# zitongbai/bipedal_control

Hardware: AMD Instinct MI355X
Metric: MPC solves/s (H1, horizon=100) (higher is better)
Workload: dtype f64; 1 GPU; Unitree H1 trot (template tiled from t = 0), horizon=100 intervals (dt 0.015), batch=256 per GPU perturbed initial states, cold start, 1 SQP iteration (BASELINE.json configs[1]); solver=sqp, global_batch=256, problems_on_rank0=256, shooting_nodes=108, nx=22, nu=22

## Files before the change

bipedal_control_amd/csrc/k_node.hip:

```cpp
#include <hip/hip_runtime.h>
#include <hip/hip_ext.h>

#include <stdexcept>

#include "kernel_launchers.h"
#include "launch.h"
#include "kernels/rollout.h"

namespace bpmpc {

template <int NJ>
__global__ __launch_bounds__(kWave) void k_prepare(Launch L) {
  constexpr int NX = 12 + NJ, NU = 12 + NJ;
  const int s = blockIdx.x, b = s / L.N, k = s % L.N;
  const int g = L.buf.p_grid[b];
  const int n = L.buf.g_nodes[g];
  if (k >= n) { if (threadIdx.x == 0) L.buf.n_info[s] = 0; return; }
  const size_t gs = (size_t)g * L.N + k;
  if (threadIdx.x == 0) L.buf.n_info[s] = 8 | ((L.buf.g_mode[gs] & 3) << 1) | (L.buf.g_kind[gs] == 1 ? 1 : 0);
  if (threadIdx.x < kNodeAux) {
    const int t = threadIdx.x;
    L.buf.n_aux[(size_t)s * kNodeAux + t] = t == 0 ? L.buf.g_dt[gs] : t < 5 ? L.buf.g_zref[gs * 4 + t - 1] : t < 9 ? L.buf.g_zdref[gs * 4 + t - 5] : 0.0;
  }
  prepare_node<NJ>(*L.model, L.buf.g_kind[gs], L.buf.g_mode[gs], L.buf.g_start[gs], L.cold != 0, k == n - 1, L.buf.p_tgt_n[b],
// ... 11 lines not shown
  if (k >= L.buf.g_nodes[L.buf.p_grid[b]]) return;
  const size_t s = sidx;
  const NodeInputs in = node_inputs<NJ>(L, b, k);
  NodeLQOut out;
  out.A = L.buf.A + s * NX * NX; out.B = L.buf.B + s * NX * NU; out.b = L.buf.b + s * NX;
  out.Q = L.buf.Q + s * NX * NX; out.R = L.buf.R + s * NU * NU; out.P = L.buf.P + s * NU * NX;
  out.q = L.buf.q + s * NX; out.r = L.buf.r + s * NU; out.c = L.buf.c + s;
  out.C = L.buf.C + s * kMaxEqRows * NX; out.D = L.buf.D + s * kMaxEqRows * NU; out.e = L.buf.e + s * kMaxEqRows;
  out.nc = L.buf.nc + s; out.perf = L.buf.perf + s * 3;
  out.prof = (b == 0 && k < 64) ? L.buf.rprof + 8 * k : nullptr;
  linearize_node<NJ>(*L.model, ws, in, out, L.ilqr != 0, L.ilqr_shift);
}

constexpr int kTrialWaves = 4;
template <int NJ> constexpr int lin_waves() { return 4; }
template <int NJ, bool MAT, bool CHAIN, bool ILQR = false>
__global__ __launch_bounds__(lin_waves<NJ>() * kWave) __attribute__((amdgpu_waves_per_eu(2, 2))) void k_linearize_fast(Launch L) {
  using C = LinFastCfg<NJ, true, CHAIN>;
  constexpr int LPN = C::LPN, NPW = C::NPW, kLinWaves = lin_waves<NJ>();
  constexpr bool PARK = sizeof(LinFastNodeLds<NJ, true, CHAIN, true>) * (kLinWaves * NPW) + sizeof(LinFastShared<NJ>) <= 80 * 1024;
  using NL = LinFastNodeLds<NJ, true, CHAIN, PARK>;
  __shared__ NL lds[kLinWaves * NPW];
  __shared__ LinFastShared<NJ> shared;
#ifdef BPMPC_LIN_TIMELINE
  const long long tl0 = wall_clock64();
#endif
  const int sub = threadIdx.x / LPN, g = threadIdx.x % LPN;
  const int widx = blockIdx.x * (kLinWaves * NPW) + sub;
  bool valid, event_wg = false;
  int b, k;
  if (L.lin_ev_n >= 0) {
    constexpr int per_wg = kLinWaves * NPW;
// ... 38 lines not shown
#endif
  valid = valid && act != 0 && info != 0;
  const size_t s = valid ? (size_t)b * L.N + k : 0;
  LinFastOut out;
  out.A = L.buf.A; out.B = L.buf.B; out.b = L.buf.b; out.Q = L.buf.Q; out.R = L.buf.R; out.q = L.buf.q; out.r = L.buf.r; out.c = L.buf.c;
  out.C = L.buf.C; out.D = L.buf.D; out.e = L.buf.e; out.perf = L.buf.perf; out.nc = L.buf.nc;
  out.park = L.buf.lin_park;
  out.dump = L.buf.lin_dump;
  out.qrd = L.buf.qrd;
  out.s = s;
  out.ilqr_shift = L.ilqr_shift;
#ifndef BPMPC_LIN_PROF_PROBLEM
#define BPMPC_LIN_PROF_PROBLEM 0
#endif
  out.prof = (valid && b == BPMPC_LIN_PROF_PROBLEM && k < 64) ? L.buf.rprof + 8 * k : nullptr;
  linearize_fast<NJ, MAT, C, NL, ILQR>(*L.model, shared, lds[sub], valid, in, pre, out, g);
#ifdef BPMPC_LIN_TIMELINE
  if (threadIdx.x % kWave == 0 && blockIdx.x < 2048) {
    double* t = L.buf.rprof + 16 * blockIdx.x + 4 * (threadIdx.x / kWave);
    unsigned hw; asm volatile("s_getreg_b32 %0, hwreg(HW_REG_HW_ID)" : "=s"(hw));
    unsigned xcc; asm volatile("s_getreg_b32 %0, hwreg(HW_REG_XCC_ID)" : "=s"(xcc));
    t[0] = (double)tl0; t[1] = (double)tl1; t[2] = (double)wall_clock64(); t[3] = (double)(hw | ((unsigned long long)(xcc & 15) << 32));
  }
#endif
}

template <int NJ>
__global__ __launch_bounds__(kWave) void k_warm_shift(Launch L, const int* restarted) {
  constexpr int NX = 12 + NJ, NU = 12 + NJ;
  __shared__ double xi[NX];
  __shared__ double Ks[2][NU * NX];
  const int b = blockIdx.x / L.N, i = blockIdx.x % L.N, l = threadIdx.x;
  const int N = L.N;
  if (restarted && restarted[b]) return;
  const int g = L.buf.p_grid[b], n = L.buf.g_nodes[g];
  if (i >= n) return;
  const int gp = L.buf.tp_grid[b], np = L.buf.tp_nodes[gp];
  if (np < 1) return;
  const double* tp = L.buf.tp_time + (size_t)gp * (N + 1);
// ... 198 lines not shown
  const size_t i0 = (size_t)blockIdx.x * blockDim.x + threadIdx.x, stride = (size_t)gridDim.x * blockDim.x;
  const double2* a2 = reinterpret_cast<const double2*>(a_src);
  const double2* b2 = reinterpret_cast<const double2*>(b_src);
  double2* ad = reinterpret_cast<double2*>(a_dst);
  double2* bd = reinterpret_cast<double2*>(b_dst);
  for (size_t i = i0; i < na / 2; i += stride) ad[i] = a2[i];
  for (size_t i = i0; i < nb / 2; i += stride) bd[i] = b2[i];
  if (i0 == 0) { if (na & 1) a_dst[na - 1] = a_src[na - 1]; if (nb & 1) b_dst[nb - 1] = b_src[nb - 1]; }
  if (iterations) for (size_t i = i0; i < (size_t)batch; i += stride) { iterations[i] = 0; active[i] = 1; }
}

namespace kl {

void prepare(int nj, int slots, hipStream_t st, const Launch& L) { KL_NJ(nj, hipLaunchKernelGGL(k_prepare<NJ>, dim3(slots), dim3(kWave), 0, st, L)); }
void linearize_reference(int nj, int slots, hipStream_t st, const Launch& L) { KL_NJ(nj, hipLaunchKernelGGL(k_linearize<NJ>, dim3(slots), dim3(kWave), 0, st, L)); }
void linearize_fast(int nj, bool materialise, int nodes, hipStream_t st, const Launch& L, hipEvent_t ev_start, hipEvent_t ev_stop) {
  KL_NJ(nj, {
    constexpr int per_wg = lin_waves<NJ>() * LinFastCfg<NJ, true>::NPW;
    const int wgs = L.lin_ev_n >= 0 ? (L.batch * L.lin_inter + per_wg - 1) / per_wg + (L.batch * L.lin_ev_n + per_wg - 1) / per_wg : (nodes + per_wg - 1) / per_wg;
    const dim3 grid(wgs), block(lin_waves<NJ>() * kWave);
    auto launch = [&](auto kernel) {
      if (ev_start && ev_stop) hipExtLaunchKernelGGL(kernel, grid, block, 0, st, ev_start, ev_stop, 0, L);
      else hipLaunchKernelGGL(kernel, grid, block, 0, st, L);
    };
    if (L.ilqr) {
      if (!L.serial_legs) throw std::runtime_error("linearize_fast: the ILQR lineariser is instantiated for serial-leg robots only");
      if (materialise) launch(k_linearize_fast<NJ, true, true, true>);
      else launch(k_linearize_fast<NJ, false, true, true>);
    } else if (L.serial_legs) {
      if (materialise) launch(k_linearize_fast<NJ, true, true>);
      else launch(k_linearize_fast<NJ, false, true>);
    } else {
      if (materialise) launch(k_linearize_fast<NJ, true, false>);
      else launch(k_linearize_fast<NJ, false, false>);
    }
  });
}
void warm_shift(int nj, int slots, hipStream_t st, const Launch& L, const int* restarted) {
  KL_NJ(nj, hipLaunchKernelGGL(k_warm_shift<NJ>, dim3(slots), dim3(kWave), 0, st, L, restarted));
}
void ls_begin(int nj, int batch, hipStream_t st, const Launch& L) { KL_NJ(nj, hipLaunchKernelGGL(k_ls_begin<NJ>, dim3(batch), dim3(kWave), 0, st, L)); }
void trial_reference(int nj, int slots, hipStream_t st, const Launch& L) { KL_NJ(nj, hipLaunchKernelGGL(k_trial<NJ>, dim3(slots), dim3(kWave), 0, st, L)); }
int trial_fast_workgroups(int nj, int nodes) {
  const int per_wg = kTrialWaves * (nj == 10 ? LinFastCfg<10, true>::NPW : LinFastCfg<12, true>::NPW);
  return (nodes + per_wg - 1) / per_wg;
}
void trial_fast(int nj, int nodes, hipStream_t st, const Launch& L) {
  const int grid = trial_fast_workgroups(nj, nodes);
  KL_NJ(nj, {
    if (L.serial_legs) hipLaunchKernelGGL((k_trial_fast<NJ, true>), dim3(grid), dim3(kTrialWaves * kWave), 0, st, L);
    else hipLaunchKernelGGL((k_trial_fast<NJ, false>), dim3(grid), dim3(kTrialWaves * kWave), 0, st, L);
  });
// ... 33 lines not shown
```

bipedal_control_amd/csrc/kernels/linearize_fast.h:

```cpp
#pragma once
#include <hip/hip_runtime.h>

#include "node_lq.h"
#include "riccati_fast.h"

namespace bpmpc {

template <int NJ, bool PACK = false, bool CHAIN_ = false>
struct LinFastCfg {
  static constexpr bool CHAIN = CHAIN_;
  static constexpr int LEG = NJ / 2;
  static constexpr int NB = NJ + 1, G = 6 + NJ, NX = 12 + NJ, NU = 12 + NJ;
  static constexpr int G0 = (PACK && G > 16 && G - 3 <= 16) ? 3 : 0;
  static constexpr int LPN = (G - G0 <= 16) ? 16 : 32;
  static constexpr int NPW = kWave / LPN;
};

struct LinFastScalars {
  double contact_off[kNumContacts][3];
  double friction, cone_reg, cone_grip, cone_shift, barrier_mu, barrier_delta, pos_gain, robot_mass;
  unsigned contact_path[kNumContacts];
  int contact_body[kNumContacts];
  int max_depth, cone_gauss_newton;
};
// ... 494 lines not shown
      acc[0] += d[1] * Fi[2] - d[2] * Fi[1];
      acc[1] += d[2] * Fi[0] - d[0] * Fi[2];
      acc[2] += d[0] * Fi[1] - d[1] * Fi[0];
    }
    const double imt = 1.0 / mass_total;
    for (int r = 0; r < 3; ++r) ev.ar_q[r] = acc[r] * imt;
  }
  }
  EVPROF(7);
}

constexpr int kLinParkDoublesPerLane = 15;
constexpr int kLinDumpNodes = 1024, kLinDumpSlack = 1024;
constexpr size_t kLinDumpDoubles = (size_t)kLinDumpNodes * 16 + kLinDumpSlack;
constexpr int kQrdStride = 40;
constexpr int kQrdRShift = 37;
constexpr int kNodeAux = 16;
constexpr int kMaxDdpSteps = 16;

struct LinFastPre {
  double x0, x1, u0, u1, xn_q, xn_h, xn_t, xr_q, xr_h, xr_t;
  double aux;
};
template <class Cfg>
__device__ __forceinline__ LinFastPre linearize_preload(const double* x, const double* xnext, const double* u, const double* xref, int ln, const double* aux = nullptr) {
  constexpr int G = Cfg::G, NX = Cfg::NX, G0 = Cfg::G0;
  const int g = ln + G0;
  const bool tr = G0 > 0 && ln < 3;
  LinFastPre p;
  p.aux = (aux && ln < kNodeAux) ? aux[ln] : 0.0;
  p.x0 = x[ln]; p.u0 = u[ln];
// ... 22 lines not shown
  static_assert(Cfg::LPN == 16 && (PACKED || Cfg::G == 16), "role slots are laid out for sixteen lanes per node");
  int ln, g;
  double* dump;
  __device__ __forceinline__ void pointers(double* Xn, double* Un, double* (&p)[NS]) const {
    if constexpr (!PACKED) {
      p[0] = Xn + (6 + ln);
      p[1] = ln < 6 ? Xn + ln : Un + (12 + ln - 6);
      p[2] = ln < 12 ? Un + ln : dump;
    } else {
      p[0] = g < Cfg::G ? Xn + (6 + g) : dump;
      p[1] = ln < 3 ? Xn + (6 + ln) : (g < Cfg::G ? Un + (12 + g - 6) : dump);
      p[2] = ln < 12 ? Un + ln : dump;
      p[3] = ln < 6 ? Xn + ln : dump;
    }
  }
  __device__ __forceinline__ void store(double* const (&p)[NS], int off, double v_coord, double v_trans, double v_mom, double v_force, double v_joint) const {
    p[0][off] = v_coord;
    if constexpr (!PACKED) {
      p[1][off] = ln < 6 ? v_mom : v_joint;
      p[2][off] = v_force;
    } else {
      p[1][off] = ln < 3 ? v_trans : v_joint;
      p[2][off] = v_force;
      p[3][off] = v_mom;
    }
  }
};

template <int NJ, bool MAT = true, class Cfg = LinFastCfg<NJ, true>, class NL = LinFastNodeLds<NJ, true, Cfg::CHAIN, false>, bool ILQR = false>
__device__ __forceinline__ void linearize_fast(const DeviceModel& md, const LinFastShared<NJ>& sh, NL& nl, bool valid,
                                               const NodeInputs& in, const LinFastPre& pre, const LinFastOut& o, int ln) {
#ifdef BPMPC_LINFAST_PROFILE
  long long lf_t[8] = {0, 0, 0, 0, 0, 0, 0, 0};
  long long lf_prev = clock64();
  const long long lf_wall0 = wall_clock64(), lf_c0 = lf_prev;
#define LFPROF(slot) do { const long long tn_ = clock64(); lf_t[slot] += tn_ - lf_prev; lf_prev = tn_; } while (0)
#else
#define LFPROF(slot) ((void)0)
#endif
  using C = Cfg;
  constexpr int G = C::G, NX = C::NX, NU = C::NU, LPN = C::LPN, G0 = C::G0;
  constexpr bool PACKED = G0 > 0;
  const int g = ln + G0;
  const bool tr = PACKED && ln < 3;
  if (!valid) return;
  if (in.kind == 1) {
    double d2 = 0.0;
    if constexpr (MAT) {
      for (int idx = ln; idx < NX * NX; idx += LPN) { (o.A + o.s * (NX * NX))[idx] = (idx / NX == idx % NX) ? 1.0 : 0.0; (o.Q + o.s * (NX * NX))[idx] = 0.0; }
      for (int idx = ln; idx < NX * NU; idx += LPN) { (o.B + o.s * (NX * NU))[idx] = 0.0; }
      for (int idx = ln; idx < NU * NU; idx += LPN) (o.R + o.s * (NU * NU))[idx] = 0.0;
      for (int idx = ln; idx < kMaxEqRows * NX; idx += LPN) (o.C + o.s * (kMaxEqRows * NX))[idx] = 0.0;
      for (int idx = ln; idx < kMaxEqRows * NU; idx += LPN) (o.D + o.s * (kMaxEqRows * NU))[idx] = 0.0;
      for (int idx = ln; idx < kMaxEqRows; idx += LPN) (o.e + o.s * (kMaxEqRows))[idx] = 0.0;
    }
    {
      static_assert(LPN == 16 && NX <= 32, "two elements of x per lane");
      const double xq_lo = __shfl(pre.x0, (6 + g) & 15, LPN), xq_hi = __shfl(pre.x1, (6 + g - 16) & 15, LPN);
      const double xq = 6 + g < 16 ? xq_lo : xq_hi;
      const double xt = __shfl(pre.x0, (6 + ln) & 15, LPN);
      if (g < G) { const double d = ILQR ? 0.0 : xq - pre.xn_q; (o.b + o.s * (NX))[6 + g] = d; d2 += d * d; }
      if (ln < 6) { const double d = ILQR ? 0.0 : pre.x0 - pre.xn_h; (o.b + o.s * (NX))[ln] = d; d2 += d * d; }
      if (tr) { const double d = ILQR ? 0.0 : xt - pre.xn_t; (o.b + o.s * (NX))[6 + ln] = d; d2 += d * d; }
      if constexpr (MAT) for (int idx = ln; idx < NX; idx += LPN) { (o.q + o.s * (NX))[idx] = 0.0; (o.r + o.s * (NU))[idx] = 0.0; }
    }
    d2 = node_allreduce_add<LPN>(d2);
// ... 178 lines not shown
    for (int rr = 3; rr < 9; ++rr) c1j[rr] = is_joint ? nl.park[9 + rr - 3][ln] : 0.0;
  } else {
    const double* pk = o.park + o.s * (15 * LPN);
    for (int rr = 0; rr < 9; ++rr) c1q[rr] = pk[rr * LPN + ln];
    for (int rr = 0; rr < 9; ++rr) c1j[rr] = 0.0;
    if (is_joint) for (int rr = 3; rr < 9; ++rr) c1j[rr] = pk[9 * LPN + (rr - 3) * LPN + ln];
  }
  for (int rr = 0; rr < 9; ++rr) {
    c1h[rr] = momentum_col(nl.X12[0], nl.X22[0], imt, mass_total, ln, rr);
    c1f[rr] = force_col(nl.cps[0], nl.com[0], imt, ln, rr);
  }
  {
    double* pab[NS];
    slots.pointers(o.A + o.s * (NX * NX), o.B + o.s * (NX * NU), pab);
#pragma unroll
    for (int r = MAT ? 0 : 3; r < (MAT ? NX : 12); ++r) {
      double aq, ah_, bf, bj;
      if (r < 3 || r >= 12) {
        aq = (r == 6 + g) ? 1.0 : 0.0;
        ah_ = (r == ln) ? 1.0 : 0.0;
        bf = (r < 3 && (ln % 3) == r) ? dt * imt : 0.0;
        bj = (r >= 12 && r == 12 + g - 6) ? dt : 0.0;
      } else if constexpr (ILQR) {
        const int rr = r - 3;
        aq = ((r == 6 + g) ? 1.0 : 0.0) + dt * c1q[rr];
        ah_ = ((r == ln) ? 1.0 : 0.0) + dt * c1h[rr];
        bf = dt * c1f[rr];
        bj = dt * c1j[rr];
      } else {
        const int rr = r - 3;
        double sq = 0.0, sh = 0.0, sf = 0.0, sj = 0.0;
        for (int l = 0; l < 9; ++l) {
          const double a = nl.a2[rr][3 + l];
          sq += a * c1q[l]; sh += a * c1h[l]; sf += a * c1f[l]; sj += a * c1j[l];
        }
        sf += nl.a2[rr][ln % 3] * imt;
        sj += e2.ar_q[rr];
        const double e2h = momentum_col(nl.X12[1], nl.X22[1], imt, mass_total, ln, rr);
        const double e2f = force_col(nl.cps[1], nl.com[1], imt, ln, rr);
        const double e2j = rr < 3 ? 0.0 : e2.br_j[rr - 3];
        aq = ((r == 6 + g) ? 1.0 : 0.0) + hdt * (c1q[rr] + e2.ar_q[rr] + dt * sq);
        ah_ = ((r == ln) ? 1.0 : 0.0) + hdt * (c1h[rr] + e2h + dt * sh);
        bf = hdt * (c1f[rr] + e2f + dt * sf);
        bj = hdt * (c1j[rr] + e2j + dt * sj);
      }
      slots.store(pab, r * NX, aq, (r == 6 + ln) ? 1.0 : 0.0, ah_, bf, bj);
      LIN_ROW_FENCE();
    }
  }
  double dyn_sse = 0.0;
  if (g < G) {
    const double v1g = NL::kPark ? nl.park[15][ln] : e1.vg;
    const double bb = ILQR ? 0.0 : nl.x[6 + g] + hdt * v1g + hdt * e2.vg - xn_q;
    (o.b + o.s * (NX))[6 + g] = bb;
    dyn_sse += bb * bb;
  }
  if (ln < 6) {
    const double bb = ILQR ? 0.0 : (ln < 6 ? xh[ln] : 0.0) + hdt * nl.fh[0][ln] + hdt * nl.fh[1][ln] - xn_h;
    (o.b + o.s * (NX))[ln] = bb;
    dyn_sse += bb * bb;
  }
  if (tr) {
    const double bb = ILQR ? 0.0 : pb[ln] + hdt * nl.vlin[0][ln] + hdt * v2t - xn_t;
// ... 8 lines not shown
  if (tr) nl.dx[6 + ln] = pt - xr_t;
  if (ln < 6) nl.dx[ln] = (ln < 6 ? xh[ln] : 0.0) - xr_h;
  if (ln < 12) nl.du[ln] = nl.u[ln] - nominal_input(sc, mode, ln);
  if (is_joint) nl.du[12 + g - 6] = ujg;
  lds_wave_sync();
  double shift = 0.0;
  for (int i = 0; i < kNumContacts; ++i)
    if (stance_flag(mode, i)) shift += -nl.cone[i][2] * sc.cone_shift;
  double cost = 0.0;
  {
    const int cq = 6 + g, ch = ln, cf = ln, cj = 12 + g - 6, ct = 6 + ln;
    const int cqs = g < G ? cq : 0, chs = ln < 6 ? ch : 0, cfs = ln < 12 ? cf : 0, cjs = is_joint ? cj : 0, cts = tr ? ct : 0;
    const bool cf_stance = ln < 12 && stance_flag(mode, cfs / 3);
    double accq = 0.0, acch = 0.0, accf = 0.0, accj = 0.0, acct = 0.0;
    double* pqr[NS];
    if constexpr (MAT) slots.pointers(o.Q + o.s * (NX * NX), o.R + o.s * (NU * NU), pqr);
#pragma unroll
    for (int r = 0; r < NX; ++r) {
      const double dxr = nl.dx[r], dur = nl.du[r];
      accq += sh.Q[cqs * NX + r] * dxr;
      if constexpr (PACKED) acct += sh.Q[cts * NX + r] * dxr;
      acch += sh.Q[chs * NX + r] * dxr;
      accf += sh.R[cfs * NU + r] * dur;
      accj += sh.R[cjs * NU + r] * dur;
      if constexpr (MAT) {
        double w = sh.R[r * NU + cfs];
        if (r == cf) w += shift;
        if (r < 12) {
          const double* cn = nl.cone[r / 3];
          const int a = r % 3, b2 = cfs % 3;
          const int lo = a < b2 ? a : b2, hi = a < b2 ? b2 : a;
          const int sidx = lo == 0 ? hi : (lo == 1 ? 2 + hi : 5);
          const double wc = w + (cn[3] * cn[4 + a] * cn[4 + b2] + cn[2] * cn[7 + sidx]);
          w = (cf_stance && r / 3 == cfs / 3) ? wc : w;
        }
        const double isf = (ILQR && r == cf) ? o.ilqr_shift : 0.0, isj = (ILQR && r == cj) ? o.ilqr_shift : 0.0;
        slots.store(pqr, r * NX, dt * (sh.Q[r * NX + cqs] + (r == cq ? shift : 0.0)), dt * (sh.Q[r * NX + cts] + (r == ct ? shift : 0.0)),
                    dt * (sh.Q[r * NX + chs] + (r == ch ? shift : 0.0)), dt * w + isf, dt * (sh.R[r * NU + cjs] + (r == cj ? shift : 0.0)) + isj);
      }
      asm volatile("" : "+v"(accq), "+v"(acch), "+v"(accf), "+v"(accj));
      if constexpr (PACKED) asm volatile("" : "+v"(acct));
      LIN_ROW_FENCE();
    }
    if (ln < 12) {
      const int blk = cf / 3, b2 = cf % 3;
      const double* cn = nl.cone[blk];
#pragma unroll
      for (int a = 0; a < 3; ++a) {
        const int r = 3 * blk + a;
        double w = sh.R[r * NU + cf];
        if (r == cf) w += shift;
        if (cf_stance) {
          const int lo = a < b2 ? a : b2, hi = a < b2 ? b2 : a;
          const int sidx = lo == 0 ? hi : (lo == 1 ? 2 + hi : 5);
          w += cn[3] * cn[4 + a] * cn[4 + b2] + cn[2] * cn[7 + sidx];
        }
        (o.qrd + o.s * kQrdStride)[1 + 3 * cf + a] = dt * w + ((ILQR && r == cf) ? o.ilqr_shift : 0.0);
      }
    }
    if (g < G) { (o.q + o.s * (NX))[cq] = dt * accq; cost += 0.5 * nl.dx[cq] * accq; }
    if (tr) { (o.q + o.s * (NX))[ct] = dt * acct; cost += 0.5 * nl.dx[ct] * acct; }
    if (ln < 6) { (o.q + o.s * (NX))[ch] = dt * acch; cost += 0.5 * nl.dx[ch] * acch; }
    if (ln < 12) {
      cost += 0.5 * nl.du[cf] * accf;
      if (stance_flag(mode, cf / 3)) accf += nl.cone[cf / 3][2] * nl.cone[cf / 3][4 + cf % 3];
      (o.r + o.s * (NU))[cf] = dt * accf;
    }
    if (is_joint) { (o.r + o.s * (NU))[cj] = dt * accj; cost += 0.5 * nl.du[cj] * accj; }
    if (ln < kNumContacts && stance_flag(mode, ln)) cost += nl.cone[ln][1];
  }
  cost = node_allreduce_add<LPN>(cost);
  dyn_sse = node_allreduce_add<LPN>(dyn_sse);
  if (ln == 0) {
    (o.qrd + o.s * kQrdStride)[0] = shift;
    if constexpr (ILQR) (o.qrd + o.s * kQrdStride)[kQrdRShift] = shift + o.ilqr_shift / dt;
    if constexpr (MAT) (o.c + o.s * (1))[0] = dt * cost;
    (o.nc + o.s * (1))[0] = nc;
    (o.perf + o.s * (3))[0] = dt * cost; (o.perf + o.s * (3))[1] = dt * dyn_sse; (o.perf + o.s * (3))[2] = dt * eq_sse;
  }
  LFPROF(5);
#ifdef BPMPC_LINFAST_PROFILE
  if (o.prof && ln == 0) {
    lf_t[6] = clock64() - lf_c0; lf_t[7] = wall_clock64() - lf_wall0;
    for (int i = 0; i < 8; ++i) o.prof[i] = (double)lf_t[i];
  }
#endif
#ifdef BPMPC_EVAL_PROFILE
  if (o.prof && ln == 0)
    for (int i = 0; i < 8; ++i) o.prof[i] = (double)evacc[i];
#endif
}
// ... 175 lines not shown
```

bipedal_control_amd/csrc/launch.h:

```cpp
#pragma once
#include <hip/hip_runtime.h>

#include <cstddef>

#include "device_model.h"
#include "kernels/linesearch.h"
#include "kernels/node_lq.h"
#include "kernels/project_node.h"
#include "kernels/riccati_fast.h"
#include "kernels/linearize_fast.h"

namespace bpmpc {

struct Buffers {
  int *g_kind, *g_mode, *g_nodes;
  double *g_dt, *g_start, *g_zref, *g_zdref;
  int* p_grid;
  double *p_x0, *p_tgt_t, *p_tgt_x;
  int* p_tgt_n;
  double *x, *u, *x_init, *u_init, *xref;
  double *A, *B, *b, *Q, *R, *P, *q, *r, *c, *C, *D, *e, *perf;
  int* nc;
  double *Px, *Pu, *Pe, *At, *Bt, *bt, *Qt, *Rt, *Pt, *qt, *rt;
  double *Wt, *Qp, *Mt;
// ... 36 lines not shown
constexpr int kLinMaxEvents = 8;
struct Launch {
  const DeviceModel* model;
  Buffers buf;
  int batch, N;
  int k0, klen;
  int cold;
  int feedback;
  int serial_legs;
  LineSearchSettings ls;
  double reg_prim;
  int lin_ev_n, lin_inter;
  int lin_ev[kLinMaxEvents];
  int ilqr;
  double ilqr_shift;
};


template <int NJ>
__device__ __forceinline__ NodeInputs node_inputs(const Launch& L, int b, int k) {
  constexpr int NX = 12 + NJ, NU = 12 + NJ;
  const int g = L.buf.p_grid[b];
  const size_t gs = (size_t)g * L.N + k, s = (size_t)b * L.N + k;
  NodeInputs in;
  in.kind = L.buf.g_kind[gs];
  in.mode = L.buf.g_mode[gs];
  in.dt = L.buf.g_dt[gs];
  in.x = L.buf.x + ((size_t)b * (L.N + 1) + k) * NX;
  in.xnext = in.x + NX;
  in.u = L.buf.u + s * NU;
// ... 93 lines not shown
```

bipedal_control_amd/csrc/solver.h:

```cpp
#pragma once
#include <hip/hip_runtime.h>

#include <algorithm>
#include <cstring>
#include <map>
#include <string>
#include <utility>
#include <vector>

#include "../../include/bpmpc.h"
#include "device_handle.h"
#include "kernel_launchers.h"
#include "launch.h"
#include "kernels/reference_device.h"

namespace bpmpc {

struct KernelTimer {
  std::vector<std::pair<hipEvent_t, hipEvent_t>> pending;
  double total_ms = 0.0;
  int launches = 0;
};

}
// ... 28 lines not shown
};

struct bpmpc_solver {
  HostStaging staging;
  PinnedArena pin_up, pin_down;
  char* xfer = nullptr;
  size_t xfer_cap = 0;
  RobotModel rm;
  DeviceModel dm;
  DeviceModel* d_model = nullptr;
  bpmpc_settings settings{};
  int nx = 0, nu = 0;
  int batch = 0, n_grids = 0, n_nodes_max = 0;
  int num_cus = 256;
  bool structured_project = false;
  int riccati_wave = 1;
  bool lin_compact = true;
  bool force_tables = false;
  bool wt_joint_rows = false;
  bool sweep_wave_regime() const { return riccati_wave == 2 || riccati_wave == 4 || ((riccati_wave == 1 || riccati_wave == 3) && batch > 2 * num_cus); }
  bool sweep_two_per_simd() const { return sweep_wave_regime() && (riccati_wave >= 3 || (riccati_wave == 1 && batch > 4 * num_cus)); }
  bool sweep_completes_joint_rows() const { return !wt_joint_rows && structured_project && !settings.reference_kernels; }
  int r8_rounds = 0;
  int eight_wave_rounds() const { return r8_rounds > 0 ? r8_rounds : (rm.nj == 10 ? 3 : 1); }
  bool sweep_eight_waves() const { return riccati_wave != 2 && riccati_wave != 4 && batch <= eight_wave_rounds() * num_cus; }
  bool has_solution = false;
  bool has_rollout = false;
  bool rollout_unchecked = false;
  double* tick_x = nullptr;
  bool loop_from_tick = false;
// ... 42 lines not shown
    L.serial_legs = (dm.serial_legs && !force_tables) ? 1 : 0;
    L.feedback = feedback();
    L.ls = ls;
    L.reg_prim = settings.reg_prim;
    L.lin_ev_n = -1; L.lin_inter = 0;
    for (int i = 0; i < kLinMaxEvents; ++i) L.lin_ev[i] = 0;
    if (n_grids == 1 && lin_compact && !grid_kind.empty() && (int)grid_nodes.size() == 1) {
      const int n = grid_nodes[0];
      int ne = 0;
      for (int k = 0; k < n; ++k)
        if (grid_kind[k] == 1) { if (ne < kLinMaxEvents) L.lin_ev[ne] = k; ++ne; }
      if (ne <= kLinMaxEvents && n == L.klen) { L.lin_ev_n = ne; L.lin_inter = n - ne; }
    }
    L.ilqr = is_ddp() ? 1 : 0;
    L.ilqr_shift = is_ddp() ? rm.ddp.ls_hessian_correction_multiple : 0.0;
    return L;
  }

  static constexpr unsigned kTimingEventFlags = hipEventDisableSystemFence;
  bool timed(const char* cls) const { return settings.profile == 1 || (settings.profile == 2 && std::strcmp(cls, "linearize") == 0); }
  void time_begin(const char* cls, hipEvent_t* a, hipEvent_t* b, hipStream_t on = nullptr) {
    if (!timed(cls)) return;
    HIP_CHECK(hipEventCreateWithFlags(a, kTimingEventFlags));
    if (hipEventCreateWithFlags(b, kTimingEventFlags) != hipSuccess) { (void)hipEventDestroy(*a); throw DeviceError("hipEventCreate failed"); }
    if (hipEventRecord(*a, on ? on : stream) != hipSuccess) { (void)hipEventDestroy(*a); (void)hipEventDestroy(*b); throw DeviceError("hipEventRecord failed"); }
  }
  void time_end(const char* cls, hipEvent_t a, hipEvent_t b, hipStream_t on = nullptr) {
    if (!timed(cls)) return;
    HIP_CHECK(hipEventRecord(b, on ? on : stream));
    KernelTimer& t = timers[cls];
// ... 106 lines not shown
```

bipedal_control_amd/csrc/solver.hip:

```cpp
#include <hip/hip_runtime.h>

#include <cmath>
#include <cstdint>
#include <algorithm>
#include <cstring>
#include <map>
#include <tuple>
#include <memory>
#include <stdexcept>
#include <string>
#include <vector>

#include "solver.h"
#include "reference_gen.h"
#include "kernels/rollout.h"

#define TIMED_ON(on, cls, ...)                                                      \
  do {                                                                              \
    hipEvent_t ev_a_, ev_b_;                                                        \
    time_begin(cls, &ev_a_, &ev_b_, on);                                            \
    __VA_ARGS__;                                                                    \
    time_end(cls, ev_a_, ev_b_, on);                                                \
    HIP_CHECK(hipGetLastError());                                                   \
  } while (0)
// ... 151 lines not shown
  a.feedback = 0;
  a.x_end = ddp.end_x; a.u_end = ddp.end_u; a.steps = ddp.roll_steps; a.status = ddp.roll_status;
  a.rec_t = ddp.rec_t; a.rec_x = ddp.rec_x; a.rec_u = ddp.rec_u; a.rec_n = ddp.rec_n; a.rec_cap = ddp.cap;
  kl::rollout(rm.nj, dm.serial_legs && !force_tables, batch, stream, d_model, a);
  kl::ddp_nominal(nj(), batch, stream, launch_params(), ddp);
  HIP_CHECK(hipGetLastError());
}

namespace {

constexpr double kDdpContractionRate = 0.5;
int ddp_step_lengths(const DdpConfig& d, int limit) {
  int n = 0;
  for (double al = d.ls_max_step_length; al >= d.ls_min_step_length && al > 0.0 && n <= limit; al *= kDdpContractionRate) ++n;
  return n;
}

void allocate(bpmpc_solver* s) {
  const size_t B = s->settings.max_batch, N = s->settings.max_nodes, NX = s->nx, NU = s->nu, S = B * N;
  Buffers& b = s->buf;
  b.qrd = s->alloc<double>("qrd", S * kQrdStride);
  b.lin_park = s->alloc<double>("lin_park", S * kLinParkDoublesPerLane * (s->rm.nj == 10 ? LinFastCfg<10, true>::LPN : LinFastCfg<12, true>::LPN));
  b.lin_dump = s->alloc<double>(nullptr, kLinDumpDoubles);
  b.x_prev = s->alloc<double>("x_prev", B * (N + 1) * NX); b.u_prev = s->alloc<double>("u_prev", S * NU);
  b.K_prev = s->alloc<double>("K_prev", S * NU * NX);
  b.tp_time = s->alloc<double>("tp_time", B * (N + 1)); b.tp_kind = s->alloc<int>("tp_kind", S, true);
  b.tp_nodes = s->alloc<int>("tp_nodes", B, true); b.tp_grid = s->alloc<int>("tp_grid", B, true);
  b.ric_carry = s->alloc<double>("ric_carry", B * (NX * NX + NX + 2));
  b.zero_page = s->alloc<double>(nullptr, 4 + 32);
  { const double one = 1.0; HIP_CHECK(hipMemcpyAsync(b.zero_page + 1, &one, sizeof(double), hipMemcpyHostToDevice, s->stream)); HIP_CHECK(hipStreamSynchronize(s->stream)); }
// ... 4 lines not shown
  b.g_time = s->alloc<double>("g_time", B * (N + 1)); b.rg_t0 = s->alloc<double>(nullptr, B); b.rg_start = s->alloc<double>(nullptr, B);
  b.p_t0 = s->alloc<double>(nullptr, B); b.p_cmd = s->alloc<double>(nullptr, B * 4); b.lib_d = s->alloc<double>(nullptr, kRefLibCapacity);
  b.rg_gait = s->alloc<int>(nullptr, B); b.rg_status = s->alloc<int>(nullptr, B); b.rg_rows = s->alloc<int>(nullptr, B); b.lib_i = s->alloc<int>(nullptr, kRefLibCapacity);
  b.g_kind = s->alloc<int>("g_kind", S, true); b.g_mode = s->alloc<int>("g_mode", S, true); b.g_nodes = s->alloc<int>("g_nodes", B, true);
  b.g_dt = s->alloc<double>("g_dt", S); b.g_start = s->alloc<double>("g_start", S);
  b.g_zref = s->alloc<double>("g_zref", S * 4); b.g_zdref = s->alloc<double>("g_zdref", S * 4);
  b.p_grid = s->alloc<int>("p_grid", B, true);
  b.p_x0 = s->alloc<double>("x0", B * NX);
  b.p_tgt_t = s->alloc<double>(nullptr, B * kMaxTargetPoints); b.p_tgt_x = s->alloc<double>(nullptr, B * kMaxTargetPoints * NX);
  b.p_tgt_n = s->alloc<int>(nullptr, B);
  b.x = s->alloc<double>("x", B * (N + 1) * NX); b.u = s->alloc<double>("u", S * NU);
  b.x_init = s->alloc<double>("x_init", B * (N + 1) * NX); b.u_init = s->alloc<double>("u_init", S * NU);
  b.xref = s->alloc<double>("xref", S * NX);
  b.A = s->alloc<double>("A", S * NX * NX); b.B = s->alloc<double>("B", S * NX * NU); b.b = s->alloc<double>("b", S * NX);
  b.Q = s->alloc<double>("Q", S * NX * NX); b.R = s->alloc<double>("R", S * NU * NU); b.P = s->alloc<double>("P", S * NU * NX);
  b.q = s->alloc<double>("q", S * NX); b.r = s->alloc<double>("r", S * NU); b.c = s->alloc<double>("c", S);
  b.C = s->alloc<double>("C", S * kMaxEqRows * NX); b.D = s->alloc<double>("D", S * kMaxEqRows * NU); b.e = s->alloc<double>("e", S * kMaxEqRows);
  b.perf = s->alloc<double>("perf", S * 3); b.nc = s->alloc<int>("nc", S, true);
  b.Px = s->alloc<double>("Px", S * NU * NX); b.Pu = s->alloc<double>("Pu", S * NU * NU); b.Pe = s->alloc<double>("Pe", S * NU);
  b.nut = s->alloc<int>("nut", S, true);
  b.n_info = s->alloc<int>("n_info", S, true);
  b.n_aux = s->alloc<double>("n_aux", S * kNodeAux);
  b.At = b.Bt = b.bt = b.Qt = b.Rt = b.Pt = b.qt = b.rt = b.Kt = b.kt = b.Wt = b.Qp = b.Mt = b.Vt = nullptr;
  if (s->settings.reference_kernels) {
    b.At = s->alloc<double>("At", S * NX * NX); b.Bt = s->alloc<double>("Bt", S * NX * NU); b.bt = s->alloc<double>("bt", S * NX);
    b.Qt = s->alloc<double>("Qt", S * NX * NX); b.Rt = s->alloc<double>("Rt", S * NU * NU); b.Pt = s->alloc<double>("Pt", S * NU * NX);
    b.qt = s->alloc<double>("qt", S * NX); b.rt = s->alloc<double>("rt", S * NU);
    b.Kt = s->alloc<double>("Kt", S * NU * NX); b.kt = s->alloc<double>("kt", S * NU);
  } else {
    const size_t wp = ((NX + 1 + NU + 15) / 16) * 16;
// ... 567 lines not shown
    s->nx = s->rm.nx; s->nu = s->rm.nu;
    HIP_CHECK(hipSetDevice(settings->device));
    { hipDeviceProp_t prop; HIP_CHECK(hipGetDeviceProperties(&prop, settings->device)); s->num_cus = prop.multiProcessorCount; }
    { const char* e = std::getenv("BPMPC_WT_JOINT_ROWS"); s->wt_joint_rows = e && e[0] == '1'; }
    { const char* e = std::getenv("BPMPC_LIN_TABLES"); s->force_tables = e && e[0] == '1'; }
    { const char* e = std::getenv("BPMPC_LIN_COMPACT"); s->lin_compact = !(e && e[0] == '0'); }
    { const char* e = std::getenv("BPMPC_RICCATI_WAVE"); s->riccati_wave = e ? std::atoi(e) : 1; }
    { const char* e = std::getenv("BPMPC_R8_ROUNDS"); s->r8_rounds = e ? std::atoi(e) : 0; }
    {
      bool block_diagonal = true;
      for (int c = 0; c < 12; ++c)
        for (int j = 12; j < s->nu; ++j) block_diagonal = block_diagonal && s->dm.R[c * s->nu + j] == 0.0 && s->dm.R[j * s->nu + c] == 0.0;
      const char* e = std::getenv("BPMPC_DENSE_PROJECT");
      s->structured_project = block_diagonal && !(e && e[0] == '1');
    }
    if (s->is_ddp() && !(s->dm.serial_legs && !s->force_tables)) s->settings.reference_kernels = 1;
    if (settings->stream) { s->stream = static_cast<hipStream_t>(settings->stream); }
    else { HIP_CHECK(hipStreamCreateWithFlags(&s->stream, hipStreamNonBlocking)); s->own_stream = true; }
    if (s->settings.pipeline_chunks <= 0) s->settings.pipeline_chunks = 1;
    if (s->settings.pipeline_chunks > 16) s->settings.pipeline_chunks = 16;
    HIP_CHECK(hipStreamCreateWithFlags(&s->producer_stream, hipStreamNonBlocking));
    HIP_CHECK(hipEventCreateWithFlags(&s->ev_go, hipEventDisableTiming));
    s->ev_chunk.resize(s->settings.pipeline_chunks);
    for (auto& e : s->ev_chunk) HIP_CHECK(hipEventCreateWithFlags(&e, hipEventDisableTiming));
    {
      std::vector<char> host(kLinImageOffset + sizeof(LinFastShared<12, true>), 0);
      std::memcpy(host.data(), &s->dm, sizeof(DeviceModel));
      if (s->rm.nj == 10) fill_shared_image<10>(s->dm, *reinterpret_cast<LinFastShared<10, true>*>(host.data() + kLinImageOffset));
      else if (s->rm.nj == 12) fill_shared_image<12>(s->dm, *reinterpret_cast<LinFastShared<12, true>*>(host.data() + kLinImageOffset));
      HIP_CHECK(hipMalloc(reinterpret_cast<void**>(&s->d_model), host.size()));
// ... 211 lines not shown
```

Measured before the change: 343,600 solves/s.

## Skip writing structurally constant rows and zeros of A, B, Q, R in lineariser

The materialising lineariser no longer rewrites the constant identity/zero rows of A and the structurally zero entries of Q and R on every call. A one-time init kernel seeds the identity diagonals of A at allocation. When the cost matrices are detected as diagonal or block-structured, new kernel variants write only the diagonal or block entries of Q and R. This cuts global memory stores per node. The risk is correctness, since it relies on unwritten entries staying zero from allocation and on downstream kernels never modifying them.

```diff
diff --git a/bipedal_control_amd/csrc/k_node.hip b/bipedal_control_amd/csrc/k_node.hip
--- a/bipedal_control_amd/csrc/k_node.hip
+++ b/bipedal_control_amd/csrc/k_node.hip
@@ -49,8 +49,8 @@
 
 constexpr int kTrialWaves = 4;
 template <int NJ> constexpr int lin_waves() { return 4; }
-template <int NJ, bool MAT, bool CHAIN, bool ILQR = false>
-__global__ __launch_bounds__(lin_waves<NJ>() * kWave) __attribute__((amdgpu_waves_per_eu(2, 2))) void k_linearize_fast(Launch L) {
+template <int NJ, bool MAT, bool CHAIN, bool ILQR, int WS>
+__device__ __forceinline__ void linearize_fast_workgroup(const Launch& L) {
   using C = LinFastCfg<NJ, true, CHAIN>;
   constexpr int LPN = C::LPN, NPW = C::NPW, kLinWaves = lin_waves<NJ>();
   constexpr bool PARK = sizeof(LinFastNodeLds<NJ, true, CHAIN, true>) * (kLinWaves * NPW) + sizeof(LinFastShared<NJ>) <= 80 * 1024;
@@ -119,7 +119,7 @@
 #define BPMPC_LIN_PROF_PROBLEM 0
 #endif
   out.prof = (valid && b == BPMPC_LIN_PROF_PROBLEM && k < 64) ? L.buf.rprof + 8 * k : nullptr;
-  linearize_fast<NJ, MAT, C, NL, ILQR>(*L.model, shared, lds[sub], valid, in, pre, out, g);
+  linearize_fast<NJ, MAT, C, NL, ILQR, WS>(*L.model, shared, lds[sub], valid, in, pre, out, g);
 #ifdef BPMPC_LIN_TIMELINE
   if (threadIdx.x % kWave == 0 && blockIdx.x < 2048) {
     double* t = L.buf.rprof + 16 * blockIdx.x + 4 * (threadIdx.x / kWave);
@@ -128,6 +128,15 @@
     t[0] = (double)tl0; t[1] = (double)tl1; t[2] = (double)wall_clock64(); t[3] = (double)(hw | ((unsigned long long)(xcc & 15) << 32));
   }
 #endif
+}
+template <int NJ, bool MAT, bool CHAIN, bool ILQR = false>
+__global__ __launch_bounds__(lin_waves<NJ>() * kWave) __attribute__((amdgpu_waves_per_eu(2, 2))) void k_linearize_fast(Launch L) {
+  linearize_fast_workgroup<NJ, MAT, CHAIN, ILQR, MAT ? (kLqSparseQ | kLqSparseR) : 0>(L);
+}
+template <int NJ, bool CHAIN, bool ILQR, int WS>
+__global__ __launch_bounds__(lin_waves<NJ>() * kWave) __attribute__((amdgpu_waves_per_eu(2, 2))) void k_linearize_fast_rows(Launch L) {
+  static_assert(WS != (kLqSparseQ | kLqSparseR), "that is k_linearize_fast");
+  linearize_fast_workgroup<NJ, true, CHAIN, ILQR, WS>(L);
 }
 
 template <int NJ>
@@ -356,6 +365,13 @@
 
 void prepare(int nj, int slots, hipStream_t st, const Launch& L) { KL_NJ(nj, hipLaunchKernelGGL(k_prepare<NJ>, dim3(slots), dim3(kWave), 0, st, L)); }
 void linearize_reference(int nj, int slots, hipStream_t st, const Launch& L) { KL_NJ(nj, hipLaunchKernelGGL(k_linearize<NJ>, dim3(slots), dim3(kWave), 0, st, L)); }
+#define LIN_MAT(...)                                                                                \
+    switch (L.lq_write_set & (kLqSparseQ | kLqSparseR)) {                                           \
+      case 0: launch(k_linearize_fast_rows<NJ, __VA_ARGS__, 0>); break;                             \
+      case kLqSparseQ: launch(k_linearize_fast_rows<NJ, __VA_ARGS__, kLqSparseQ>); break;           \
+      case kLqSparseR: launch(k_linearize_fast_rows<NJ, __VA_ARGS__, kLqSparseR>); break;           \
+      default: launch(k_linearize_fast<NJ, true, __VA_ARGS__>); break;                              \
+    }
 void linearize_fast(int nj, bool materialise, int nodes, hipStream_t st, const Launch& L, hipEvent_t ev_start, hipEvent_t ev_stop) {
   KL_NJ(nj, {
     constexpr int per_wg = lin_waves<NJ>() * LinFastCfg<NJ, true>::NPW;
@@ -367,17 +383,18 @@
     };
     if (L.ilqr) {
       if (!L.serial_legs) throw std::runtime_error("linearize_fast: the ILQR lineariser is instantiated for serial-leg robots only");
-      if (materialise) launch(k_linearize_fast<NJ, true, true, true>);
+      if (materialise) { LIN_MAT(true, true) }
       else launch(k_linearize_fast<NJ, false, true, true>);
     } else if (L.serial_legs) {
-      if (materialise) launch(k_linearize_fast<NJ, true, true>);
+      if (materialise) { LIN_MAT(true, false) }
       else launch(k_linearize_fast<NJ, false, true>);
     } else {
-      if (materialise) launch(k_linearize_fast<NJ, true, false>);
+      if (materialise) { LIN_MAT(false, false) }
       else launch(k_linearize_fast<NJ, false, false>);
     }
   });
 }
+#undef LIN_MAT
 void warm_shift(int nj, int slots, hipStream_t st, const Launch& L, const int* restarted) {
   KL_NJ(nj, hipLaunchKernelGGL(k_warm_shift<NJ>, dim3(slots), dim3(kWave), 0, st, L, restarted));
 }
diff --git a/bipedal_control_amd/csrc/kernels/linearize_fast.h b/bipedal_control_amd/csrc/kernels/linearize_fast.h
--- a/bipedal_control_amd/csrc/kernels/linearize_fast.h
+++ b/bipedal_control_amd/csrc/kernels/linearize_fast.h
@@ -532,7 +532,9 @@
 constexpr int kLinDumpNodes = 1024, kLinDumpSlack = 1024;
 constexpr size_t kLinDumpDoubles = (size_t)kLinDumpNodes * 16 + kLinDumpSlack;
 constexpr int kQrdStride = 40;
+constexpr int kQrdWriteSet = 38;
 constexpr int kQrdRShift = 37;
+constexpr int kLqSparseQ = 1, kLqSparseR = 2;
 constexpr int kNodeAux = 16;
 constexpr int kMaxDdpSteps = 16;
 
@@ -585,6 +587,12 @@
       p[3] = ln < 6 ? Xn + ln : dump;
     }
   }
+  __device__ __forceinline__ void pointers(double* Xn, double* Un, double* (&p)[NS], bool drop_x, bool drop_u) const {
+    pointers(Xn, Un, p);
+    const bool s1x = PACKED ? ln < 3 : ln < 6;
+    if (drop_x) { p[0] = dump; if (s1x) p[1] = dump; if constexpr (PACKED) p[3] = dump; }
+    if (drop_u) { p[2] = dump; if (!s1x) p[1] = dump; }
+  }
   __device__ __forceinline__ void store(double* const (&p)[NS], int off, double v_coord, double v_trans, double v_mom, double v_force, double v_joint) const {
     p[0][off] = v_coord;
     if constexpr (!PACKED) {
@@ -598,7 +606,7 @@
   }
 };
 
-template <int NJ, bool MAT = true, class Cfg = LinFastCfg<NJ, true>, class NL = LinFastNodeLds<NJ, true, Cfg::CHAIN, false>, bool ILQR = false>
+template <int NJ, bool MAT = true, class Cfg = LinFastCfg<NJ, true>, class NL = LinFastNodeLds<NJ, true, Cfg::CHAIN, false>, bool ILQR = false, int WS = 0>
 __device__ __forceinline__ void linearize_fast(const DeviceModel& md, const LinFastShared<NJ>& sh, NL& nl, bool valid,
                                                const NodeInputs& in, const LinFastPre& pre, const LinFastOut& o, int ln) {
 #ifdef BPMPC_LINFAST_PROFILE
@@ -618,9 +626,15 @@
   if (in.kind == 1) {
     double d2 = 0.0;
     if constexpr (MAT) {
-      for (int idx = ln; idx < NX * NX; idx += LPN) { (o.A + o.s * (NX * NX))[idx] = (idx / NX == idx % NX) ? 1.0 : 0.0; (o.Q + o.s * (NX * NX))[idx] = 0.0; }
-      for (int idx = ln; idx < NX * NU; idx += LPN) { (o.B + o.s * (NX * NU))[idx] = 0.0; }
-      for (int idx = ln; idx < NU * NU; idx += LPN) (o.R + o.s * (NU * NU))[idx] = 0.0;
+      for (int idx = 3 * NX + ln; idx < 12 * NX; idx += LPN) { (o.A + o.s * (NX * NX))[idx] = (idx / NX == idx % NX) ? 1.0 : 0.0; (o.B + o.s * (NX * NU))[idx] = 0.0; }
+      if (ln < 12) (o.B + o.s * (NX * NU))[(ln % 3) * NU + ln] = 0.0;
+      for (int j = ln; j < NJ; j += LPN) (o.B + o.s * (NX * NU))[(12 + j) * NU + 12 + j] = 0.0;
+      if constexpr (WS & kLqSparseQ) { for (int idx = ln; idx < NX; idx += LPN) (o.Q + o.s * (NX * NX))[idx * NX + idx] = 0.0; }
+      else { for (int idx = ln; idx < NX * NX; idx += LPN) (o.Q + o.s * (NX * NX))[idx] = 0.0; }
+      if constexpr (WS & kLqSparseR) {
+        for (int idx = ln; idx < 9 * kNumContacts; idx += LPN) (o.R + o.s * (NU * NU))[(3 * (idx / 9) + (idx % 9) / 3) * NU + 3 * (idx / 9) + idx % 3] = 0.0;
+        for (int idx = ln; idx < NJ * NJ; idx += LPN) (o.R + o.s * (NU * NU))[(12 + idx / NJ) * NU + 12 + idx % NJ] = 0.0;
+      } else { for (int idx = ln; idx < NU * NU; idx += LPN) (o.R + o.s * (NU * NU))[idx] = 0.0; }
       for (int idx = ln; idx < kMaxEqRows * NX; idx += LPN) (o.C + o.s * (kMaxEqRows * NX))[idx] = 0.0;
       for (int idx = ln; idx < kMaxEqRows * NU; idx += LPN) (o.D + o.s * (kMaxEqRows * NU))[idx] = 0.0;
       for (int idx = ln; idx < kMaxEqRows; idx += LPN) (o.e + o.s * (kMaxEqRows))[idx] = 0.0;
@@ -829,14 +843,9 @@
     double* pab[NS];
     slots.pointers(o.A + o.s * (NX * NX), o.B + o.s * (NX * NU), pab);
 #pragma unroll
-    for (int r = MAT ? 0 : 3; r < (MAT ? NX : 12); ++r) {
+    for (int r = 3; r < 12; ++r) {
       double aq, ah_, bf, bj;
-      if (r < 3 || r >= 12) {
-        aq = (r == 6 + g) ? 1.0 : 0.0;
-        ah_ = (r == ln) ? 1.0 : 0.0;
-        bf = (r < 3 && (ln % 3) == r) ? dt * imt : 0.0;
-        bj = (r >= 12 && r == 12 + g - 6) ? dt : 0.0;
-      } else if constexpr (ILQR) {
+      if constexpr (ILQR) {
         const int rr = r - 3;
         aq = ((r == 6 + g) ? 1.0 : 0.0) + dt * c1q[rr];
         ah_ = ((r == ln) ? 1.0 : 0.0) + dt * c1h[rr];
@@ -862,6 +871,13 @@
       slots.store(pab, r * NX, aq, (r == 6 + ln) ? 1.0 : 0.0, ah_, bf, bj);
       LIN_ROW_FENCE();
     }
+    if constexpr (MAT) {
+      double* Bn = o.B + o.s * (NX * NU);
+      double* pf = ln < 12 ? Bn + ((ln % 3) * NU + ln) : slots.dump;
+      double* pj = is_joint ? Bn + ((12 + g - 6) * NU + 12 + g - 6) : slots.dump;
+      *pf = dt * imt;
+      *pj = dt;
+    }
   }
   double dyn_sse = 0.0;
   if (g < G) {
@@ -900,7 +916,10 @@
     const bool cf_stance = ln < 12 && stance_flag(mode, cfs / 3);
     double accq = 0.0, acch = 0.0, accf = 0.0, accj = 0.0, acct = 0.0;
     double* pqr[NS];
-    if constexpr (MAT) slots.pointers(o.Q + o.s * (NX * NX), o.R + o.s * (NU * NU), pqr);
+    constexpr bool SQ = MAT && (WS & kLqSparseQ) != 0, SR = MAT && (WS & kLqSparseR) != 0;
+    constexpr bool QR_ROWS = MAT && !(SQ && SR);
+    if constexpr (QR_ROWS) slots.pointers(o.Q + o.s * (NX * NX), o.R + o.s * (NU * NU), pqr, SQ, SR);
+    double* const pjr = !SR ? nullptr : (is_joint ? o.R + o.s * (NU * NU) + cjs : slots.dump);
 #pragma unroll
     for (int r = 0; r < NX; ++r) {
       const double dxr = nl.dx[r], dur = nl.du[r];
@@ -909,7 +928,7 @@
       acch += sh.Q[chs * NX + r] * dxr;
       accf += sh.R[cfs * NU + r] * dur;
       accj += sh.R[cjs * NU + r] * dur;
-      if constexpr (MAT) {
+      if constexpr (QR_ROWS) {
         double w = sh.R[r * NU + cfs];
         if (r == cf) w += shift;
         if (r < 12) {
@@ -924,6 +943,9 @@
         slots.store(pqr, r * NX, dt * (sh.Q[r * NX + cqs] + (r == cq ? shift : 0.0)), dt * (sh.Q[r * NX + cts] + (r == ct ? shift : 0.0)),
                     dt * (sh.Q[r * NX + chs] + (r == ch ? shift : 0.0)), dt * w + isf, dt * (sh.R[r * NU + cjs] + (r == cj ? shift : 0.0)) + isj);
       }
+      if constexpr (SR) {
+        if (r >= 12) { const double isj = (ILQR && r == cj) ? o.ilqr_shift : 0.0; pjr[r * NU] = dt * (sh.R[r * NU + cjs] + (r == cj ? shift : 0.0)) + isj; }
+      }
       asm volatile("" : "+v"(accq), "+v"(acch), "+v"(accf), "+v"(accj));
       if constexpr (PACKED) asm volatile("" : "+v"(acct));
       LIN_ROW_FENCE();
@@ -941,12 +963,14 @@
           const int sidx = lo == 0 ? hi : (lo == 1 ? 2 + hi : 5);
           w += cn[3] * cn[4 + a] * cn[4 + b2] + cn[2] * cn[7 + sidx];
         }
-        (o.qrd + o.s * kQrdStride)[1 + 3 * cf + a] = dt * w + ((ILQR && r == cf) ? o.ilqr_shift : 0.0);
-      }
-    }
-    if (g < G) { (o.q + o.s * (NX))[cq] = dt * accq; cost += 0.5 * nl.dx[cq] * accq; }
-    if (tr) { (o.q + o.s * (NX))[ct] = dt * acct; cost += 0.5 * nl.dx[ct] * acct; }
-    if (ln < 6) { (o.q + o.s * (NX))[ch] = dt * acch; cost += 0.5 * nl.dx[ch] * acch; }
+        const double v = dt * w + ((ILQR && r == cf) ? o.ilqr_shift : 0.0);
+        (o.qrd + o.s * kQrdStride)[1 + 3 * cf + a] = v;
+        if constexpr (SR) (o.R + o.s * (NU * NU))[r * NU + cf] = v;
+      }
+    }
+    if (g < G) { (o.q + o.s * (NX))[cq] = dt * accq; if constexpr (SQ) (o.Q + o.s * (NX * NX))[cq * NX + cq] = dt * (sh.Q[cq * NX + cq] + shift); cost += 0.5 * nl.dx[cq] * accq; }
+    if (tr) { (o.q + o.s * (NX))[ct] = dt * acct; if constexpr (SQ) (o.Q + o.s * (NX * NX))[ct * NX + ct] = dt * (sh.Q[ct * NX + ct] + shift); cost += 0.5 * nl.dx[ct] * acct; }
+    if (ln < 6) { (o.q + o.s * (NX))[ch] = dt * acch; if constexpr (SQ) (o.Q + o.s * (NX * NX))[ch * NX + ch] = dt * (sh.Q[ch * NX + ch] + shift); cost += 0.5 * nl.dx[ch] * acch; }
     if (ln < 12) {
       cost += 0.5 * nl.du[cf] * accf;
       if (stance_flag(mode, cf / 3)) accf += nl.cone[cf / 3][2] * nl.cone[cf / 3][4 + cf % 3];
@@ -960,7 +984,7 @@
   if (ln == 0) {
     (o.qrd + o.s * kQrdStride)[0] = shift;
     if constexpr (ILQR) (o.qrd + o.s * kQrdStride)[kQrdRShift] = shift + o.ilqr_shift / dt;
-    if constexpr (MAT) (o.c + o.s * (1))[0] = dt * cost;
+    if constexpr (MAT) { (o.c + o.s * (1))[0] = dt * cost; (o.qrd + o.s * kQrdStride)[kQrdWriteSet] = (double)WS; }
     (o.nc + o.s * (1))[0] = nc;
     (o.perf + o.s * (3))[0] = dt * cost; (o.perf + o.s * (3))[1] = dt * dyn_sse; (o.perf + o.s * (3))[2] = dt * eq_sse;
   }
diff --git a/bipedal_control_amd/csrc/launch.h b/bipedal_control_amd/csrc/launch.h
--- a/bipedal_control_amd/csrc/launch.h
+++ b/bipedal_control_amd/csrc/launch.h
@@ -74,6 +74,7 @@
   int lin_ev[kLinMaxEvents];
   int ilqr;
   double ilqr_shift;
+  int lq_write_set;
 };
 
 
diff --git a/bipedal_control_amd/csrc/solver.h b/bipedal_control_amd/csrc/solver.h
--- a/bipedal_control_amd/csrc/solver.h
+++ b/bipedal_control_amd/csrc/solver.h
@@ -66,6 +66,7 @@
   int batch = 0, n_grids = 0, n_nodes_max = 0;
   int num_cus = 256;
   bool structured_project = false;
+  int lq_write_set = 0;
   int riccati_wave = 1;
   bool lin_compact = true;
   bool force_tables = false;
@@ -138,6 +139,7 @@
     }
     L.ilqr = is_ddp() ? 1 : 0;
     L.ilqr_shift = is_ddp() ? rm.ddp.ls_hessian_correction_multiple : 0.0;
+    L.lq_write_set = lq_write_set;
     return L;
   }
 
diff --git a/bipedal_control_amd/csrc/solver.hip b/bipedal_control_amd/csrc/solver.hip
--- a/bipedal_control_amd/csrc/solver.hip
+++ b/bipedal_control_amd/csrc/solver.hip
@@ -189,6 +189,28 @@
   int n = 0;
   for (double al = d.ls_max_step_length; al >= d.ls_min_step_length && al > 0.0 && n <= limit; al *= kDdpContractionRate) ++n;
   return n;
+}
+
+__global__ __launch_bounds__(256) void k_init_structural_rows(double* A, size_t slots, int nx) {
+  const int per = nx - 9;
+  const size_t i = (size_t)blockIdx.x * 256 + threadIdx.x;
+  if (i >= slots * (size_t)per) return;
+  const size_t s = i / per;
+  const int j = (int)(i % per), r = j < 3 ? j : j + 9;
+  A[s * (size_t)nx * nx + (size_t)r * nx + r] = 1.0;
+}
+
+int lq_write_set_of(const DeviceModel& dm, int nx, int nu) {
+  auto zero = [](double v) { return v == 0.0 && !std::signbit(v); };
+  bool q_diagonal = true, r_structured = true;
+  for (int r = 0; r < nx; ++r)
+    for (int c = 0; c < nx; ++c) q_diagonal = q_diagonal && (r == c || zero(dm.Q[r * nx + c]));
+  for (int r = 0; r < nu; ++r)
+    for (int c = 0; c < nu; ++c) {
+      const bool written = (r < 12 && c < 12 && r / 3 == c / 3) || (r >= 12 && c >= 12);
+      r_structured = r_structured && (written || zero(dm.R[r * nu + c]));
+    }
+  return (q_diagonal ? kLqSparseQ : 0) | (r_structured ? kLqSparseR : 0);
 }
 
 void allocate(bpmpc_solver* s) {
@@ -223,6 +245,11 @@
   b.xref = s->alloc<double>("xref", S * NX);
   b.A = s->alloc<double>("A", S * NX * NX); b.B = s->alloc<double>("B", S * NX * NU); b.b = s->alloc<double>("b", S * NX);
   b.Q = s->alloc<double>("Q", S * NX * NX); b.R = s->alloc<double>("R", S * NU * NU); b.P = s->alloc<double>("P", S * NU * NX);
+  {
+    const size_t n = S * (NX - 9);
+    hipLaunchKernelGGL(k_init_structural_rows, dim3((unsigned)((n + 255) / 256)), dim3(256), 0, s->stream, b.A, S, (int)NX);
+    HIP_CHECK(hipGetLastError());
+  }
   b.q = s->alloc<double>("q", S * NX); b.r = s->alloc<double>("r", S * NU); b.c = s->alloc<double>("c", S);
   b.C = s->alloc<double>("C", S * kMaxEqRows * NX); b.D = s->alloc<double>("D", S * kMaxEqRows * NU); b.e = s->alloc<double>("e", S * kMaxEqRows);
   b.perf = s->alloc<double>("perf", S * 3); b.nc = s->alloc<int>("nc", S, true);
@@ -820,6 +847,7 @@
       const char* e = std::getenv("BPMPC_DENSE_PROJECT");
       s->structured_project = block_diagonal && !(e && e[0] == '1');
     }
+    { const char* e = std::getenv("BPMPC_LQ_FULL_ROWS"); s->lq_write_set = (e && e[0] == '1') ? 0 : lq_write_set_of(s->dm, s->nx, s->nu); }
     if (s->is_ddp() && !(s->dm.serial_legs && !s->force_tables)) s->settings.reference_kernels = 1;
     if (settings->stream) { s->stream = static_cast<hipStream_t>(settings->stream); }
     else { HIP_CHECK(hipStreamCreateWithFlags(&s->stream, hipStreamNonBlocking)); s->own_stream = true; }
```

After: 346,200 solves/s, median of 6. About the same (+0.7%).
